# TThuraya/multimodal-PL

Measured on AMD Instinct MI355X. Metric: train voxels/sec at 96^3 patch, 1/2/4/8 MI355X; fwd+bwd step ms, higher is better.
Workload: dtype bf16; 1 GPU; unet3D_baseline([1,2,2,2,2],16,weight_std) fwd+EDiceLoss_partial+bwd+SGD; model=unet3D_baseline-16, global_batch=2, seq_len=884736, parallelism=dp1, world_size_seen=1, force_buckets=False

## Files before the change

multimodal-pl_amd/csrc/conv_brick_gen.hip:

```cpp
#include "common.h"

namespace u3d {

typedef __attribute__((ext_vector_type(8))) __bf16 bf16x8;

constexpr int GB_BD = 4, GB_BH = 8, GB_BW = 16;
constexpr int GB_HD = GB_BD + 2, GB_HH = GB_BH + 2, GB_HW = GB_BW + 2;
constexpr int GB_NH = GB_HD * GB_HH * GB_HW;
constexpr int GB_NT = 512;
constexpr int GB_HLD = (GB_NH + GB_NT / 4 - 1) / (GB_NT / 4);
constexpr int GB_PS = GB_NH * 16 + 64;
constexpr int GB_MAXN = 16;
constexpr int GB_MAXC = 256;

struct GBGeom {
  int n, d, h, w;
  int cin, cout, cin_p, cout_p;
  int nbd, nbh, nbw;
  int gn_groups;
  int nct;
  float* fstats;
  unsigned* fcnt;
};

__device__ __forceinline__ int gb_seg(int r) {
  return (r < 4 || (r >= 12 && r < 16) || (r >= 20 && r < 28)) ? 0 : 1;
}
__device__ __forceinline__ int gb_pos(int r) {
  if (r < 4) return r;
  if (r < 12) return r - 4;
  if (r < 16) return r - 8;
  if (r < 20) return r - 8;
  if (r < 28) return r - 12;
  return r - 16;
}

template <int CO, bool FLIP>
__global__ __launch_bounds__(GB_NT, 1) void convg_brick_kernel(const bf16* __restrict__ x, const bf16* __restrict__ wpk,
                                                              bf16* __restrict__ y, const bf16* __restrict__ res,
                                                              const float* __restrict__ gstat,
                                                              const float* __restrict__ gamma,
                                                              const float* __restrict__ beta, GBGeom g) {
  constexpr int TN = CO / 32;
  constexpr int WROWS = 9 * CO;
  constexpr int WLD = (WROWS * 4 + GB_NT - 1) / GB_NT;
  __shared__ __attribute__((aligned(16))) char hal[4 * GB_PS];
  __shared__ __attribute__((aligned(16))) char wbuf[2][4 * WROWS * 16];

  const int tid = threadIdx.x, lane = tid & 63, wave = tid >> 6;
  const int r = lane & 31, hh = lane >> 5;
  const int nwg = gridDim.x, nct = g.nct;
  int bid;
  {
    const int q = nwg >> 3, rr = nwg & 7, xcd = blockIdx.x & 7, loc = blockIdx.x >> 3;
    bid = (xcd < rr ? xcd * (q + 1) : rr * (q + 1) + (xcd - rr) * q) + loc;
  }
  int b = bid / nct;
  const int bw_ = b % g.nbw; b /= g.nbw;
  const int bh_ = b % g.nbh; b /= g.nbh;
  const int bd_ = b % g.nbd;
  const int nn = b / g.nbd;
  const int d0 = bd_ * GB_BD, h0 = bh_ * GB_BH, w0 = bw_ * GB_BW;
  const int co0 = (bid - (bid / nct) * nct) * CO;
  const bool has_gn = gstat != nullptr;
  const int nchunk = g.cin_p / 32;
  const int nsteps = nchunk * 3;

  u32x4 hpre[GB_HLD];
  u32x4 wpre[WLD];

  const int sch = tid & 3, srow0 = tid >> 2;
  f32x2 sc[4], sh[4];
  auto halo_load = [&](int c) {
#pragma unroll
    for (int i = 0; i < GB_HLD; ++i) {
      const int row = srow0 + i * (GB_NT / 4);
      u32x4 v = {0u, 0u, 0u, 0u};
      if (row < GB_NH) {
        const int hw = row % GB_HW, hr = (row / GB_HW) % GB_HH, hd = row / (GB_HW * GB_HH);
        const int zd = d0 - 1 + hd, zh = h0 - 1 + hr, zw = w0 - 1 + hw;
        const int cc = c * 32 + sch * 8;
        if ((unsigned)zd < (unsigned)g.d && (unsigned)zh < (unsigned)g.h && (unsigned)zw < (unsigned)g.w && cc < g.cin)
          v = *reinterpret_cast<const u32x4*>(x + ((((long long)nn * g.d + zd) * g.h + zh) * g.w + zw) * g.cin + cc);
      }
      hpre[i] = v;
    }
  };
  auto gn_table = [&](int c) {
    if (has_gn) gn_coef8(gstat, gamma, beta, g.gn_groups, g.cin, nn, c * 32 + sch * 8, sc, sh);
  };
  auto halo_commit = [&]() {
#pragma unroll
    for (int i = 0; i < GB_HLD; ++i) {
      const int row = srow0 + i * (GB_NT / 4);
      if (row < GB_NH) {
        u32x4 v = hpre[i];
        if (has_gn) {
          const int hw = row % GB_HW, hr = (row / GB_HW) % GB_HH, hd = row / (GB_HW * GB_HH);
          const int zd = d0 - 1 + hd, zh = h0 - 1 + hr, zw = w0 - 1 + hw;
          if ((unsigned)zd < (unsigned)g.d && (unsigned)zh < (unsigned)g.h && (unsigned)zw < (unsigned)g.w)
            v = gn_relu8(v, sc, sh);
        }
        *reinterpret_cast<u32x4*>(hal + sch * GB_PS + row * 16) = v;
      }
    }
  };
  auto w_load = [&](int s) {
    const int c = s / 3, td = s % 3;
#pragma unroll
    for (int i = 0; i < WLD; ++i) {
      const int ci = tid + i * GB_NT;
      u32x4 v = {0u, 0u, 0u, 0u};
      if (ci < WROWS * 4) {
        const int ch = ci / WROWS, row = ci % WROWS;
        const int j = row / CO, co = co0 + row % CO;
        const int t = td * 9 + j;
        if (co < g.cout_p)
          v = *reinterpret_cast<const u32x4*>(wpk + ((long long)t * g.cout_p + co) * g.cin_p + c * 32 + ch * 8);
      }
      wpre[i] = v;
    }
  };
  auto w_commit = [&](int buf) {
#pragma unroll
    for (int i = 0; i < WLD; ++i) {
      const int ci = tid + i * GB_NT;
      if (ci < WROWS * 4) {
        const int ch = ci / WROWS, row = ci % WROWS;
        *reinterpret_cast<u32x4*>(wbuf[buf] + (ch * WROWS + row) * 16) = wpre[i];
      }
    }
  };

  gn_table(0);
  halo_load(0);
  w_load(0);
  __syncthreads();
  halo_commit();
  w_commit(0);
  __syncthreads();

  f32x16 acc[2][TN];
#pragma unroll
  for (int tm = 0; tm < 2; ++tm)
#pragma unroll
    for (int tn = 0; tn < TN; ++tn)
#pragma unroll
      for (int e = 0; e < 16; ++e) acc[tm][tn][e] = 0.f;

  int arow[2];
#pragma unroll
  for (int tm = 0; tm < 2; ++tm) {
    const int rt = 2 * wave + tm, vd = rt >> 2, vh = 2 * (rt & 3) + gb_seg(r);
    arow[tm] = (vd * GB_HH + vh) * GB_HW + gb_pos(r);
  }

  for (int s = 0; s < nsteps; ++s) {
    const int td = s % 3;
    const bool last_plane = td == 2;
    if (s + 1 < nsteps) w_load(s + 1);
    if (last_plane && s + 1 < nsteps) halo_load(s / 3 + 1);
    const char* wb = wbuf[s & 1];
    const int od = FLIP ? 2 - td : td;
#pragma unroll 3
    for (int j = 0; j < 9; ++j) {
      const int th = j / 3, tw = j % 3;
      const int oh = FLIP ? 2 - th : th, ow = FLIP ? 2 - tw : tw;
      const int toff = (od * GB_HH + oh) * GB_HW + ow;
#pragma unroll
      for (int k = 0; k < 2; ++k) {
        const int plane = 2 * k + hh;
        bf16x8 a[2], bb[TN];
#pragma unroll
        for (int tm = 0; tm < 2; ++tm)
          a[tm] = *reinterpret_cast<const bf16x8*>(hal + plane * GB_PS + (arow[tm] + toff) * 16);
#pragma unroll
        for (int tn = 0; tn < TN; ++tn)
          bb[tn] = *reinterpret_cast<const bf16x8*>(wb + (plane * WROWS + j * CO + tn * 32 + r) * 16);
#pragma unroll
        for (int tm = 0; tm < 2; ++tm)
#pragma unroll
          for (int tn = 0; tn < TN; ++tn)
            acc[tm][tn] = __builtin_amdgcn_mfma_f32_32x32x16_bf16(a[tm], bb[tn], acc[tm][tn], 0, 0, 0);
      }
    }
    if (s + 1 < nsteps) {
      w_commit((s + 1) & 1);
      if (last_plane) {
        gn_table(s / 3 + 1);
        __syncthreads();
        halo_commit();
      }
    }
    __syncthreads();
  }

  constexpr int VB = CO * 2;
  char* const ept = hal + wave * (2 * 32 * VB);
  u32x4 rv[2][VB / 32];
  long long obase[2];
  bool dok[2];
#pragma unroll
  for (int tm = 0; tm < 2; ++tm) {
    const int rt = 2 * wave + tm, zd = d0 + (rt >> 2);
    dok[tm] = zd < g.d;
    obase[tm] = (((long long)nn * g.d + zd) * g.h + h0 + 2 * (rt & 3)) * g.w + w0;
  }
  auto chunk_ok = [&](int tm, int q, long long& off) {
    const int v = q / (VB / 16), c = q % (VB / 16);
    const int seg = v >> 4, pos = v & 15;
    const int rt = 2 * wave + tm, zh = h0 + 2 * (rt & 3) + seg, zw = w0 + pos, co = co0 + c * 8;
    off = (obase[tm] + (long long)seg * g.w + pos) * g.cout + co;
    return dok[tm] && zh < g.h && zw < g.w && co < g.cout;
  };
  if (res) {
#pragma unroll
    for (int tm = 0; tm < 2; ++tm)
#pragma unroll
      for (int u = 0; u < VB / 32; ++u) {
        long long off;
        rv[tm][u] = chunk_ok(tm, lane + 64 * u, off) ? *reinterpret_cast<const u32x4*>(res + off)
                                                      : u32x4{0u, 0u, 0u, 0u};
      }
  }
#pragma unroll
  for (int tm = 0; tm < 2; ++tm)
#pragma unroll
    for (int tn = 0; tn < TN; ++tn)
#pragma unroll
      for (int i = 0; i < 16; ++i) {
        const int ri = (i & 3) + 8 * (i >> 2) + 4 * hh;
        const int v = gb_seg(ri) * 16 + gb_pos(ri);
        *reinterpret_cast<bf16*>(ept + (tm * 32 + v) * VB + (tn * 32 + r) * 2) = from_f<bf16>(acc[tm][tn][i]);
      }
  __builtin_amdgcn_wave_barrier();
  asm volatile("" ::: "memory");
#pragma unroll
  for (int tm = 0; tm < 2; ++tm)
#pragma unroll
    for (int u = 0; u < VB / 32; ++u) {
      const int q = lane + 64 * u;
      long long off;
      if (!chunk_ok(tm, q, off)) continue;
      u32x4 v = *reinterpret_cast<const u32x4*>(ept + tm * 32 * VB + q * 16);
      if (res) {
        float a[8], c[8];
        load16<bf16>(reinterpret_cast<const bf16*>(&v), a);
        load16<bf16>(reinterpret_cast<const bf16*>(&rv[tm][u]), c);
#pragma unroll
        for (int e = 0; e < 8; ++e) a[e] += c[e];
        store16<bf16>(reinterpret_cast<bf16*>(&v), a);
      }
      *reinterpret_cast<u32x4*>(y + off) = v;
    }
}

template <int CO, bool FLIP, int BWX = 16, bool GB = false>
__global__ __launch_bounds__(GB_NT, 1) void convg_pbrick_kernel(const bf16* __restrict__ x, const bf16* __restrict__ wpk,
                                                               bf16* __restrict__ y, const bf16* __restrict__ res,
                                                               const float* __restrict__ gstat,
                                                               const float* __restrict__ gamma,
                                                               const float* __restrict__ beta, GBGeom g, int per,
                                                               int nunits, float* __restrict__ spart = nullptr) {
  constexpr int TN = CO / 32;
  constexpr int WROWS = 9 * CO;
  constexpr int WLD = (WROWS * 4 + GB_NT - 1) / GB_NT;
  constexpr int BW = BWX, HH = GB_BH + 2, HW = BW + 2, NH = (GB_BD + 2) * HH * HW;
  constexpr int HLD = (NH + GB_NT / 4 - 1) / (GB_NT / 4), PS = NH * 16 + 64, TM = BW / 8;
  static_assert(BW == 16 || BW == 8, "brick width");
  auto tile_vox = [](int rt, int r, int& vd, int& vh, int& vw) {
    if constexpr (BW == 16) {
      vd = rt >> 2; vh = 2 * (rt & 3) + gb_seg(r); vw = gb_pos(r);
    } else {
      vd = rt >> 1; vh = 4 * (rt & 1) + (r >> 3); vw = r & 7;
    }
  };
  __shared__ __attribute__((aligned(16))) char hal[4 * PS];
  constexpr int WPS = WROWS * 16 + 64;
  __shared__ __attribute__((aligned(16))) char wbuf[2][4 * WPS];
  __shared__ __attribute__((aligned(16))) f32x2 gtab[2][GB_MAXC];
  __shared__ __attribute__((aligned(16))) f32x4 gbt[GB ? 2 : 1][GB ? GB_MAXC : 1];
  __shared__ double sst[8][2][TN * 2 * 4][2];

  static_assert(!GB || FLIP, "GB: data gradient only");
  constexpr int GB_EARLY = TM == 1 ? TN : 1;
  if constexpr (FLIP && !GB) {
    res = nullptr;
    spart = nullptr;
  }
  float* const gbpart = GB ? spart : nullptr;
  if constexpr (GB) spart = nullptr;
  const int tid = threadIdx.x, lane = tid & 63, wave = tid >> 6;
  const int r = lane & 31, hh = lane >> 5;
  int bid;
  {
    const int nwg = gridDim.x, q = nwg >> 3, rr = nwg & 7, xcd = blockIdx.x & 7, loc = blockIdx.x >> 3;
    bid = (xcd < rr ? xcd * (q + 1) : rr * (q + 1) + (xcd - rr) * q) + loc;
  }
  const int u_begin = bid * per, u_end = min(nunits, u_begin + per);
  const int nct = g.nct;
  const bool has_gn = gstat != nullptr;
  const bool pro_gn = !FLIP && has_gn;
  const int gtc = FLIP ? g.cout : g.cin, gtc_p = FLIP ? g.cout_p : g.cin_p;
  const int nchunk = g.cin_p / 32;
  const int nsteps = nchunk * 3;

  struct Unit {
    int nn, d0, h0, w0, co0;
  };
  auto unit_geo = [&](int u) {
    Unit q;
    int b = u / nct;
    q.co0 = (u - b * nct) * CO;
    const int bw_ = b % g.nbw; b /= g.nbw;
    const int bh_ = b % g.nbh; b /= g.nbh;
    const int bd_ = b % g.nbd;
    q.nn = b / g.nbd;
    q.d0 = bd_ * GB_BD; q.h0 = bh_ * GB_BH; q.w0 = bw_ * BW;
    return q;
  };

  u32x4 hpre[HLD];
  unsigned hmask = 0;
  u32x4 wpre[WLD];
  const int sch = tid & 3, srow0 = tid >> 2;
  int stg_nn = 0, stg_c = 0;
  const auto srs = __builtin_amdgcn_make_buffer_rsrc((void*)gstat, 0, has_gn ? 0x7FFFFFFF : 0, 0x00020000);
  const auto grs = __builtin_amdgcn_make_buffer_rsrc((void*)gamma, 0, has_gn ? 0x7FFFFFFF : 0, 0x00020000);
  const auto brs = __builtin_amdgcn_make_buffer_rsrc((void*)beta, 0, has_gn ? 0x7FFFFFFF : 0, 0x00020000);
  auto gtab_fill = [&](int nn) {
    if (has_gn && tid < gtc_p) {
      int t = tid;
      asm volatile("" : "+v"(t));
      const int c = min(t, gtc - 1), gg = c / (gtc / g.gn_groups);
      const int so = (nn * g.gn_groups + gg) * 8;
      const float mean = __builtin_bit_cast(float, __builtin_amdgcn_raw_buffer_load_b32(srs, so, 0, 0));
      const float rstd = __builtin_bit_cast(float, __builtin_amdgcn_raw_buffer_load_b32(srs, so + 4, 0, 0));
      const float sc_ = rstd * __builtin_bit_cast(float, __builtin_amdgcn_raw_buffer_load_b32(grs, c * 4, 0, 0));
      const float sh_ = __builtin_bit_cast(float, __builtin_amdgcn_raw_buffer_load_b32(brs, c * 4, 0, 0)) - mean * sc_;
      if constexpr (GB)
        gbt[nn & 1][tid] = f32x4{sc_, sh_, rstd, mean};
      else
        gtab[nn & 1][tid] = f32x2{sc_, sh_};
    }
  };
  const int xbytes = g.n * g.d * g.h * g.w * g.cin * 2, ybytes = g.n * g.d * g.h * g.w * g.cout * 2;
  const auto xrs = __builtin_amdgcn_make_buffer_rsrc((void*)x, 0, xbytes, 0x00020000);
  const auto wrs = __builtin_amdgcn_make_buffer_rsrc((void*)wpk, 0, 27 * g.cout_p * g.cin_p * 2, 0x00020000);
  const auto rrs = __builtin_amdgcn_make_buffer_rsrc((void*)res, 0, res ? ybytes : 0, 0x00020000);
  const auto yrs = __builtin_amdgcn_make_buffer_rsrc((void*)y, 0, ybytes, 0x00020000);
  const auto prs = __builtin_amdgcn_make_buffer_rsrc((void*)spart, 0, spart ? 0x7FFFFFFF : 0, 0x00020000);
  auto halo_load = [&](const Unit& q, int c) {
    hmask = 0;
    stg_nn = q.nn;
    stg_c = c;
    const int cc = c * 32 + sch * 8;
#pragma unroll
    for (int i = 0; i < HLD; ++i) {
      const int row = srow0 + i * (GB_NT / 4);
      const int hw = row % HW, hr = (row / HW) % HH, hd = row / (HW * HH);
      const int zd = q.d0 - 1 + hd, zh = q.h0 - 1 + hr, zw = q.w0 - 1 + hw;
      const bool in = row < NH && (unsigned)zd < (unsigned)g.d && (unsigned)zh < (unsigned)g.h &&
                      (unsigned)zw < (unsigned)g.w;
      hmask |= (in ? 1u : 0u) << i;
      const unsigned off =
          in && cc < g.cin ? (unsigned)(((((q.nn * g.d + zd) * g.h + zh) * g.w + zw) * g.cin + cc) * 2) : 0xFFFFFFF0u;
      hpre[i] = __builtin_bit_cast(u32x4, __builtin_amdgcn_raw_buffer_load_b128(xrs, off, 0, 0));
    }
  };
  auto halo_commit = [&]() {
    f32x2 sc[4], sh[4];
    if (pro_gn) {
      const f32x2* t = &gtab[stg_nn & 1][stg_c * 32 + sch * 8];
#pragma unroll
      for (int e = 0; e < 4; ++e) {
        const f32x2 a0 = t[2 * e], a1 = t[2 * e + 1];
        sc[e] = f32x2{a0[0], a1[0]};
        sh[e] = f32x2{a0[1], a1[1]};
      }
    }
#pragma unroll
    for (int i = 0; i < HLD; ++i) {
      const int row = srow0 + i * (GB_NT / 4);
      if (row < NH) {
        u32x4 v = hpre[i];
        if (pro_gn && ((hmask >> i) & 1u)) v = gn_relu8(v, sc, sh);
        *reinterpret_cast<u32x4*>(hal + sch * PS + row * 16) = v;
      }
    }
  };
  auto w_load = [&](int co0, int s) {
    const int c = s / 3, td = s % 3;
#pragma unroll
    for (int i = 0; i < WLD; ++i) {
      const int ci = tid + i * GB_NT;
      const int ch = ci & 3, row = ci >> 2;
      const int j = row / CO, co = co0 + row % CO;
      const int t = td * 9 + j;
      const unsigned off = ci < WROWS * 4 && co < g.cout_p
                               ? (unsigned)(((t * g.cout_p + co) * g.cin_p + c * 32 + ch * 8) * 2) : 0xFFFFFFF0u;
      wpre[i] = __builtin_bit_cast(u32x4, __builtin_amdgcn_raw_buffer_load_b128(wrs, off, 0, 0));
    }
  };
// ... 397 lines not shown

static bool pbrick_bw8(int w) {
  const int e8 = opt(OPT_CONVG_BW8);
  return e8 >= 0 ? e8 != 0 : (w % 16 != 0 && w % 8 == 0);
}

static bool gb_co64(long long units, int cout, int cout_p) {
  const int env_co32 = opt(OPT_CONVG_CO32);
  if (cout_p < 64 || env_co32 == 1) return false;
  return !(env_co32 < 0 && units * cdiv(cout, 64) < 128 && units * cdiv(cout, 32) >= 128);
}

struct GBPlan {
  bool pers, bw8, co64;
  int nunits, per, nwg;
};

static GBPlan gb_plan(bool flip, int n, int cin, int d, int h, int w, int cout, bool gn, bool residual, bool gbparts,
                      GBGeom& g) {
  g = GBGeom{};
  g.n = n; g.d = d; g.h = h; g.w = w;
  g.cin = cin; g.cout = cout; g.cin_p = round_up(cin, 32); g.cout_p = round_up(cout, 32);
  GBPlan p{};
  p.pers = opt(OPT_CONVG_PERSIST) != 0 && n >= 1 && n <= GB_MAXN &&
           fits_buffer_offsets((long long)n * d * h * w * std::max(cin, cout) * 2) &&
           fits_buffer_offsets(27LL * g.cout_p * g.cin_p * 2) &&
           (!gn || (gbparts ? g.cout_p : g.cin_p) <= GB_MAXC) && !(flip && residual);
  p.bw8 = p.pers && pbrick_bw8(w);
  g.nbd = cdiv(d, GB_BD); g.nbh = cdiv(h, GB_BH); g.nbw = cdiv(w, p.bw8 ? 8 : GB_BW);
  const long long bricks = (long long)n * g.nbd * g.nbh * g.nbw;
  p.co64 = gb_co64(bricks, cout, g.cout_p);
  g.nct = cdiv(cout, p.co64 ? 64 : 32);
  p.nunits = (int)(bricks * g.nct);
  p.per = p.pers ? cdiv(p.nunits, convg_num_cus()) : 1;
  p.nwg = cdiv(p.nunits, p.per);
  return p;
}

extern "C" long long u3d_convg_brick_stats_ws_floats(int n, int d, int h, int w, int cout) {
  return (long long)n * cdiv(d, GB_BD) * cdiv(h, GB_BH) * cdiv(w, 8) * cdiv(cout, 32) * 128;
}

struct GBArgs {
  const void *x, *wpk;
  void* y;
  const void* res;
  const float *gstat, *gamma, *beta;
  float* spart;
  hipStream_t s;
};

template <int CO, bool FLIP, int BWX, bool GB>
static void gb_launch(const GBPlan& p, const GBGeom& g, const GBArgs& a) {
  if (p.pers)
    hipLaunchKernelGGL((convg_pbrick_kernel<CO, FLIP, BWX, GB>), dim3(p.nwg), dim3(GB_NT), 0, a.s, (const bf16*)a.x,
                       (const bf16*)a.wpk, (bf16*)a.y, (const bf16*)a.res, a.gstat, a.gamma, a.beta, g, p.per, p.nunits,
                       a.spart);
  else
    hipLaunchKernelGGL((convg_brick_kernel<CO, FLIP>), dim3(p.nwg), dim3(GB_NT), 0, a.s, (const bf16*)a.x,
                       (const bf16*)a.wpk, (bf16*)a.y, (const bf16*)a.res, a.gstat, a.gamma, a.beta, g);
}

template <int CO>
static void gb_dispatch(bool flip, bool gb, const GBPlan& p, const GBGeom& g, const GBArgs& a) {
  if (!flip) p.bw8 ? gb_launch<CO, false, 8, false>(p, g, a) : gb_launch<CO, false, 16, false>(p, g, a);
  else if (gb) p.bw8 ? gb_launch<CO, true, 8, true>(p, g, a) : gb_launch<CO, true, 16, true>(p, g, a);
  else p.bw8 ? gb_launch<CO, true, 8, false>(p, g, a) : gb_launch<CO, true, 16, false>(p, g, a);
}

static int convg_impl(int flip, const void* x, int n, int cin, int d, int h, int w, const void* wpk, int cout,
                      const float* gn_stats, const float* gn_gamma, const float* gn_beta, int gn_groups,
                      const void* residual, void* y, float* spart, float* stats_out, u3d_stream_t stream,
                      const void* gbx = nullptr, float* gbparts = nullptr, unsigned* fcnt = nullptr) {
  U3D_REQUIRE(x && wpk && y && n >= 1 && n <= GB_MAXN, "convg_brick: bad args");
  U3D_REQUIRE(!gbparts || (flip && gbx && gn_stats && !residual && !spart && cout % gn_groups == 0),
              "convg_brick_dgrad_gn: bad args");
  U3D_REQUIRE(cin % 8 == 0 && cout % 8 == 0, "convg_brick: channels must be multiples of 8");
  U3D_REQUIRE(!gn_stats || (gn_gamma && gn_beta && gn_groups > 0 && (gbparts ? cout : cin) % gn_groups == 0),
              "convg_brick: bad GN");
  GBGeom g;
  const GBPlan p = gb_plan(flip, n, cin, d, h, w, cout, gn_stats, residual, gbparts, g);
  g.gn_groups = gn_groups;
  U3D_REQUIRE(!spart || (p.pers && !flip && cout % 32 == 0), "convg_brick_stats: needs the persistent forward, cout %% 32 == 0");
  U3D_REQUIRE(!gbparts || p.pers, "convg_brick_dgrad_gn: needs the persistent data gradient (u3d_convg_brick_gn_nparts)");
  if (spart && fcnt) {
    g.fstats = stats_out;
    g.fcnt = fcnt;
  }
  hipStream_t s = (hipStream_t)stream;
  const GBArgs a{x, wpk, y, gbparts ? gbx : residual, gn_stats, gn_gamma, gn_beta, gbparts ? gbparts : spart, s};
  if (p.co64) gb_dispatch<64>(flip, gbparts, p, g, a);
  else gb_dispatch<32>(flip, gbparts, p, g, a);
  int rc = check_launch(p.pers ? "convg_pbrick_kernel" : "convg_brick_kernel");
  if (rc || !spart || fcnt) return rc;
  hipLaunchKernelGGL(pbrick_gn_finalize_kernel, dim3(n * 16), dim3(256), 0, s, (const double*)spart, p.co64 ? 64 : 32, g.nct,
                     g.nbd * g.nbh * g.nbw, cout, (double)(cout / 16) * d * h * w, stats_out);
  return check_launch("pbrick_gn_finalize_kernel");
}

extern "C" int u3d_convg_brick(int flip, const void* x, int n, int cin, int d, int h, int w, const void* wpk, int cout,
                               const float* gn_stats, const float* gn_gamma, const float* gn_beta, int gn_groups,
                               const void* residual, void* y, u3d_stream_t stream) {
  return convg_impl(flip, x, n, cin, d, h, w, wpk, cout, gn_stats, gn_gamma, gn_beta, gn_groups, residual, y, nullptr,
                    nullptr, stream);
}

extern "C" int u3d_convg_brick_gn_nparts(int n, int cin, int d, int h, int w, int cout) {
  GBGeom g;
// ... 33 lines not shown
```

Before: 336.6 million voxels/s.

## Switch brick conv kernels to 16x16x32 MFMA with swizzled LDS layout

Reworks the brick convolution kernels to use 16x16x32 bf16 MFMA tiles instead of 32x32x16. Each wave now covers four rows of 16 voxels, and the halo and weight LDS buffers get padded or XOR-swizzled strides to cut bank conflicts. The epilogue and the GroupNorm stats reduction are rewritten around the new fragment layout, using permlane swaps and bpermute trees. The old 32x32 path is kept as a separate kernel for the 8-wide bricks. This is a large change that risks register pressure and correctness problems in the new reduction paths.

Result: no change. 338.4 million voxels/s, median of 6 (+0.5%).

```diff
diff --git a/multimodal-pl_amd/csrc/conv_brick_gen.hip b/multimodal-pl_amd/csrc/conv_brick_gen.hip
--- a/multimodal-pl_amd/csrc/conv_brick_gen.hip
+++ b/multimodal-pl_amd/csrc/conv_brick_gen.hip
@@ -9,7 +9,8 @@
 constexpr int GB_NH = GB_HD * GB_HH * GB_HW;
 constexpr int GB_NT = 512;
 constexpr int GB_HLD = (GB_NH + GB_NT / 4 - 1) / (GB_NT / 4);
-constexpr int GB_PS = GB_NH * 16 + 64;
+constexpr int gb_plane_stride(int nh) { return (nh * 16 + 255) / 256 * 256 + 32; }
+constexpr int GB_PS = gb_plane_stride(GB_NH);
 constexpr int GB_MAXN = 16;
 constexpr int GB_MAXC = 256;
 
@@ -23,16 +24,48 @@
   unsigned* fcnt;
 };
 
-__device__ __forceinline__ int gb_seg(int r) {
-  return (r < 4 || (r >= 12 && r < 16) || (r >= 20 && r < 28)) ? 0 : 1;
-}
-__device__ __forceinline__ int gb_pos(int r) {
-  if (r < 4) return r;
-  if (r < 12) return r - 4;
-  if (r < 16) return r - 8;
-  if (r < 20) return r - 8;
-  if (r < 28) return r - 12;
-  return r - 16;
+__device__ __forceinline__ int gb_m16(int l16) { return (l16 >= 4 && l16 < 12) ? 2 * (l16 - 4) : 2 * (l16 & 7) + 1; }
+
+__device__ __forceinline__ int gb_wswz(int plane) { return 2 * (plane & 1) + 12 * (plane >> 1); }
+
+template <int NV, int NC, int LD>
+__device__ __forceinline__ void gb_mfma_tap(f32x4 (*acc)[LD], int c0, const bf16x8 (&fw)[NC], const bf16x8 (&fx)[NV]) {
+#pragma unroll
+  for (int v = 0; v < NV; ++v)
+#pragma unroll
+    for (int cb = 0; cb < NC; ++cb)
+      acc[v][c0 + cb] = __builtin_amdgcn_mfma_f32_16x16x32_bf16(fw[cb], fx[v], acc[v][c0 + cb], 0, 0, 0);
+}
+
+__device__ __forceinline__ int gb_cbase(int q4) { return 16 * (q4 & 1) + 8 * (q4 >> 1); }
+__device__ __forceinline__ u32x4 gb_pack_pair(const f32x4& a0, const f32x4& a1) {
+  uint32_t pk[2][2] = {{pack_bf16x2(a0[0], a0[1]), pack_bf16x2(a0[2], a0[3])},
+                       {pack_bf16x2(a1[0], a1[1]), pack_bf16x2(a1[2], a1[3])}};
+#pragma unroll
+  for (int e = 0; e < 2; ++e) {
+    const auto sw = __builtin_amdgcn_permlane16_swap(pk[0][e], pk[1][e], false, false);
+    pk[0][e] = sw[0];
+    pk[1][e] = sw[1];
+  }
+  return u32x4{pk[0][0], pk[0][1], pk[1][0], pk[1][1]};
+}
+
+__device__ __forceinline__ void gb_tree_lanes(int lane, int m, int (&px)[5]) {
+  constexpr int C[5] = {8, 12, 4, 2, 1};
+#pragma unroll
+  for (int k = 0; k < 5; ++k) {
+    const int t = m ^ C[k], h = t >> 1;
+    px[k] = ((lane & 48) + ((t & 1) ? (h < 4 ? h : h + 8) : h + 4)) * 4;
+  }
+}
+__device__ __forceinline__ float gb_bperm(int addr, float v) {
+  return __builtin_bit_cast(float, __builtin_amdgcn_ds_bpermute(addr, __builtin_bit_cast(int, v)));
+}
+__device__ __forceinline__ float gb_wave_tree(float y0, float y1, const int (&px)[5]) {
+  float t = y0 + gb_bperm(px[0], y1);
+#pragma unroll
+  for (int k = 1; k < 5; ++k) t += gb_bperm(px[k], t);
+  return t;
 }
 
 template <int CO, bool FLIP>
@@ -41,14 +74,14 @@
                                                               const float* __restrict__ gstat,
                                                               const float* __restrict__ gamma,
                                                               const float* __restrict__ beta, GBGeom g) {
-  constexpr int TN = CO / 32;
+  constexpr int NVB = 4, NCB = CO / 16;
   constexpr int WROWS = 9 * CO;
   constexpr int WLD = (WROWS * 4 + GB_NT - 1) / GB_NT;
   __shared__ __attribute__((aligned(16))) char hal[4 * GB_PS];
   __shared__ __attribute__((aligned(16))) char wbuf[2][4 * WROWS * 16];
 
   const int tid = threadIdx.x, lane = tid & 63, wave = tid >> 6;
-  const int r = lane & 31, hh = lane >> 5;
+  const int l16 = lane & 15, q4 = lane >> 4;
   const int nwg = gridDim.x, nct = g.nct;
   int bid;
   {
@@ -140,20 +173,13 @@
   w_commit(0);
   __syncthreads();
 
-  f32x16 acc[2][TN];
-#pragma unroll
-  for (int tm = 0; tm < 2; ++tm)
-#pragma unroll
-    for (int tn = 0; tn < TN; ++tn)
-#pragma unroll
-      for (int e = 0; e < 16; ++e) acc[tm][tn][e] = 0.f;
-
-  int arow[2];
-#pragma unroll
-  for (int tm = 0; tm < 2; ++tm) {
-    const int rt = 2 * wave + tm, vd = rt >> 2, vh = 2 * (rt & 3) + gb_seg(r);
-    arow[tm] = (vd * GB_HH + vh) * GB_HW + gb_pos(r);
-  }
+  f32x4 acc[NVB][NCB];
+#pragma unroll
+  for (int vb = 0; vb < NVB; ++vb)
+#pragma unroll
+    for (int cb = 0; cb < NCB; ++cb) acc[vb][cb] = f32x4{0.f, 0.f, 0.f, 0.f};
+
+  const int xrow = ((wave >> 1) * GB_HH + 4 * (wave & 1)) * GB_HW + gb_m16(l16);
 
   for (int s = 0; s < nsteps; ++s) {
     const int td = s % 3;
@@ -167,22 +193,14 @@
       const int th = j / 3, tw = j % 3;
       const int oh = FLIP ? 2 - th : th, ow = FLIP ? 2 - tw : tw;
       const int toff = (od * GB_HH + oh) * GB_HW + ow;
-#pragma unroll
-      for (int k = 0; k < 2; ++k) {
-        const int plane = 2 * k + hh;
-        bf16x8 a[2], bb[TN];
-#pragma unroll
-        for (int tm = 0; tm < 2; ++tm)
-          a[tm] = *reinterpret_cast<const bf16x8*>(hal + plane * GB_PS + (arow[tm] + toff) * 16);
-#pragma unroll
-        for (int tn = 0; tn < TN; ++tn)
-          bb[tn] = *reinterpret_cast<const bf16x8*>(wb + (plane * WROWS + j * CO + tn * 32 + r) * 16);
-#pragma unroll
-        for (int tm = 0; tm < 2; ++tm)
-#pragma unroll
-          for (int tn = 0; tn < TN; ++tn)
-            acc[tm][tn] = __builtin_amdgcn_mfma_f32_32x32x16_bf16(a[tm], bb[tn], acc[tm][tn], 0, 0, 0);
-      }
+      bf16x8 fx[NVB], fw[NCB];
+#pragma unroll
+      for (int vb = 0; vb < NVB; ++vb)
+        fx[vb] = *reinterpret_cast<const bf16x8*>(hal + q4 * GB_PS + (xrow + toff + vb * GB_HW) * 16);
+#pragma unroll
+      for (int cb = 0; cb < NCB; ++cb)
+        fw[cb] = *reinterpret_cast<const bf16x8*>(wb + (q4 * WROWS + j * CO + cb * 16 + l16) * 16);
+      gb_mfma_tap<NVB, NCB>(acc, 0, fw, fx);
     }
     if (s + 1 < nsteps) {
       w_commit((s + 1) & 1);
@@ -196,63 +214,51 @@
   }
 
   constexpr int VB = CO * 2;
-  char* const ept = hal + wave * (2 * 32 * VB);
-  u32x4 rv[2][VB / 32];
-  long long obase[2];
-  bool dok[2];
-#pragma unroll
-  for (int tm = 0; tm < 2; ++tm) {
-    const int rt = 2 * wave + tm, zd = d0 + (rt >> 2);
-    dok[tm] = zd < g.d;
-    obase[tm] = (((long long)nn * g.d + zd) * g.h + h0 + 2 * (rt & 3)) * g.w + w0;
-  }
-  auto chunk_ok = [&](int tm, int q, long long& off) {
-    const int v = q / (VB / 16), c = q % (VB / 16);
-    const int seg = v >> 4, pos = v & 15;
-    const int rt = 2 * wave + tm, zh = h0 + 2 * (rt & 3) + seg, zw = w0 + pos, co = co0 + c * 8;
-    off = (obase[tm] + (long long)seg * g.w + pos) * g.cout + co;
-    return dok[tm] && zh < g.h && zw < g.w && co < g.cout;
+  constexpr int NCH = VB / 16;
+  char* const ept = hal + wave * (64 * VB);
+  u32x4 rv[NCH];
+  const int zd = d0 + (wave >> 1), zh0 = h0 + 4 * (wave & 1);
+  const long long obase = (((long long)nn * g.d + zd) * g.h + zh0) * g.w + w0;
+  auto chunk_ok = [&](int q, long long& off) {
+    const int v = q / NCH, c = q % NCH;
+    const int vb = v >> 4, pos = v & 15, co = co0 + c * 8;
+    off = (obase + (long long)vb * g.w + pos) * g.cout + co;
+    return zd < g.d && zh0 + vb < g.h && w0 + pos < g.w && co < g.cout;
   };
   if (res) {
 #pragma unroll
-    for (int tm = 0; tm < 2; ++tm)
-#pragma unroll
-      for (int u = 0; u < VB / 32; ++u) {
-        long long off;
-        rv[tm][u] = chunk_ok(tm, lane + 64 * u, off) ? *reinterpret_cast<const u32x4*>(res + off)
-                                                      : u32x4{0u, 0u, 0u, 0u};
-      }
-  }
-#pragma unroll
-  for (int tm = 0; tm < 2; ++tm)
-#pragma unroll
-    for (int tn = 0; tn < TN; ++tn)
-#pragma unroll
-      for (int i = 0; i < 16; ++i) {
-        const int ri = (i & 3) + 8 * (i >> 2) + 4 * hh;
-        const int v = gb_seg(ri) * 16 + gb_pos(ri);
-        *reinterpret_cast<bf16*>(ept + (tm * 32 + v) * VB + (tn * 32 + r) * 2) = from_f<bf16>(acc[tm][tn][i]);
-      }
+    for (int u = 0; u < NCH; ++u) {
+      long long off;
+      rv[u] = chunk_ok(lane + 64 * u, off) ? *reinterpret_cast<const u32x4*>(res + off) : u32x4{0u, 0u, 0u, 0u};
+    }
+  }
+  const int m16 = gb_m16(l16);
+#pragma unroll
+  for (int vb = 0; vb < NVB; ++vb)
+#pragma unroll
+    for (int cb = 0; cb < NCB; ++cb) {
+      const f32x4 a = acc[vb][cb];
+      *reinterpret_cast<uint2*>(ept + (vb * 16 + m16) * VB + (cb * 16 + 4 * q4) * 2) =
+          uint2{pack_bf16x2(a[0], a[1]), pack_bf16x2(a[2], a[3])};
+    }
   __builtin_amdgcn_wave_barrier();
   asm volatile("" ::: "memory");
 #pragma unroll
-  for (int tm = 0; tm < 2; ++tm)
-#pragma unroll
-    for (int u = 0; u < VB / 32; ++u) {
-      const int q = lane + 64 * u;
-      long long off;
-      if (!chunk_ok(tm, q, off)) continue;
-      u32x4 v = *reinterpret_cast<const u32x4*>(ept + tm * 32 * VB + q * 16);
-      if (res) {
-        float a[8], c[8];
-        load16<bf16>(reinterpret_cast<const bf16*>(&v), a);
-        load16<bf16>(reinterpret_cast<const bf16*>(&rv[tm][u]), c);
-#pragma unroll
-        for (int e = 0; e < 8; ++e) a[e] += c[e];
-        store16<bf16>(reinterpret_cast<bf16*>(&v), a);
-      }
-      *reinterpret_cast<u32x4*>(y + off) = v;
-    }
+  for (int u = 0; u < NCH; ++u) {
+    const int q = lane + 64 * u;
+    long long off;
+    if (!chunk_ok(q, off)) continue;
+    u32x4 v = *reinterpret_cast<const u32x4*>(ept + q * 16);
+    if (res) {
+      float a[8], c[8];
+      load16<bf16>(reinterpret_cast<const bf16*>(&v), a);
+      load16<bf16>(reinterpret_cast<const bf16*>(&rv[u]), c);
+#pragma unroll
+      for (int e = 0; e < 8; ++e) a[e] += c[e];
+      store16<bf16>(reinterpret_cast<bf16*>(&v), a);
+    }
+    *reinterpret_cast<u32x4*>(y + off) = v;
+  }
 }
 
 template <int CO, bool FLIP, int BWX = 16, bool GB = false>
@@ -262,28 +268,25 @@
                                                                const float* __restrict__ gamma,
                                                                const float* __restrict__ beta, GBGeom g, int per,
                                                                int nunits, float* __restrict__ spart = nullptr) {
-  constexpr int TN = CO / 32;
+  constexpr int TN = CO / 32, NCB = CO / 16;
   constexpr int WROWS = 9 * CO;
   constexpr int WLD = (WROWS * 4 + GB_NT - 1) / GB_NT;
   constexpr int BW = BWX, HH = GB_BH + 2, HW = BW + 2, NH = (GB_BD + 2) * HH * HW;
-  constexpr int HLD = (NH + GB_NT / 4 - 1) / (GB_NT / 4), PS = NH * 16 + 64, TM = BW / 8;
-  static_assert(BW == 16 || BW == 8, "brick width");
-  auto tile_vox = [](int rt, int r, int& vd, int& vh, int& vw) {
-    if constexpr (BW == 16) {
-      vd = rt >> 2; vh = 2 * (rt & 3) + gb_seg(r); vw = gb_pos(r);
-    } else {
-      vd = rt >> 1; vh = 4 * (rt & 1) + (r >> 3); vw = r & 7;
-    }
+  constexpr int HLD = (NH + GB_NT / 4 - 1) / (GB_NT / 4), PS = gb_plane_stride(NH), NVB = BW / 4, NVH = NVB / 2;
+  static_assert(BW == 16, "brick width");
+  auto tile_vox = [](int wave, int vb, int m, int& vd, int& vh, int& vw) {
+    vd = wave >> 1; vh = 4 * (wave & 1) + vb; vw = m;
   };
   __shared__ __attribute__((aligned(16))) char hal[4 * PS];
-  constexpr int WPS = WROWS * 16 + 64;
+  constexpr int WPS = WROWS * 16;
+  static_assert(WPS % 256 == 0 && WROWS % 16 == 0, "weight plane stride / swizzle blocks");
   __shared__ __attribute__((aligned(16))) char wbuf[2][4 * WPS];
   __shared__ __attribute__((aligned(16))) f32x2 gtab[2][GB_MAXC];
   __shared__ __attribute__((aligned(16))) f32x4 gbt[GB ? 2 : 1][GB ? GB_MAXC : 1];
-  __shared__ double sst[8][2][TN * 2 * 4][2];
+  __shared__ double sst[8][4][TN * 4][2];
 
   static_assert(!GB || FLIP, "GB: data gradient only");
-  constexpr int GB_EARLY = TM == 1 ? TN : 1;
+  constexpr int GB_EARLY = 1;
   if constexpr (FLIP && !GB) {
     res = nullptr;
     spart = nullptr;
@@ -291,7 +294,7 @@
   float* const gbpart = GB ? spart : nullptr;
   if constexpr (GB) spart = nullptr;
   const int tid = threadIdx.x, lane = tid & 63, wave = tid >> 6;
-  const int r = lane & 31, hh = lane >> 5;
+  const int l16 = lane & 15, q4 = lane >> 4, m16 = gb_m16(l16), cbase = gb_cbase(q4);
   int bid;
   {
     const int nwg = gridDim.x, q = nwg >> 3, rr = nwg & 7, xcd = blockIdx.x & 7, loc = blockIdx.x >> 3;
@@ -349,6 +352,472 @@
   const auto wrs = __builtin_amdgcn_make_buffer_rsrc((void*)wpk, 0, 27 * g.cout_p * g.cin_p * 2, 0x00020000);
   const auto rrs = __builtin_amdgcn_make_buffer_rsrc((void*)res, 0, res ? ybytes : 0, 0x00020000);
   const auto yrs = __builtin_amdgcn_make_buffer_rsrc((void*)y, 0, ybytes, 0x00020000);
+  float* const pbase = GB ? gbpart : spart;
+  const auto prs = __builtin_amdgcn_make_buffer_rsrc((void*)pbase, 0, pbase ? 0x7FFFFFFF : 0, 0x00020000);
+  auto halo_load = [&](const Unit& q, int c) {
+    hmask = 0;
+    stg_nn = q.nn;
+    stg_c = c;
+    const int cc = c * 32 + sch * 8;
+#pragma unroll
+    for (int i = 0; i < HLD; ++i) {
+      const int row = srow0 + i * (GB_NT / 4);
+      const int hw = row % HW, hr = (row / HW) % HH, hd = row / (HW * HH);
+      const int zd = q.d0 - 1 + hd, zh = q.h0 - 1 + hr, zw = q.w0 - 1 + hw;
+      const bool in = row < NH && (unsigned)zd < (unsigned)g.d && (unsigned)zh < (unsigned)g.h &&
+                      (unsigned)zw < (unsigned)g.w;
+      hmask |= (in ? 1u : 0u) << i;
+      const unsigned off =
+          in && cc < g.cin ? (unsigned)(((((q.nn * g.d + zd) * g.h + zh) * g.w + zw) * g.cin + cc) * 2) : 0xFFFFFFF0u;
+      hpre[i] = __builtin_bit_cast(u32x4, __builtin_amdgcn_raw_buffer_load_b128(xrs, off, 0, 0));
+    }
+  };
+  auto halo_commit = [&]() {
+    f32x2 sc[4], sh[4];
+    if (pro_gn) {
+      const f32x2* t = &gtab[stg_nn & 1][stg_c * 32 + sch * 8];
+#pragma unroll
+      for (int e = 0; e < 4; ++e) {
+        const f32x2 a0 = t[2 * e], a1 = t[2 * e + 1];
+        sc[e] = f32x2{a0[0], a1[0]};
+        sh[e] = f32x2{a0[1], a1[1]};
+      }
+    }
+#pragma unroll
+    for (int i = 0; i < HLD; ++i) {
+      const int row = srow0 + i * (GB_NT / 4);
+      if (row < NH) {
+        u32x4 v = hpre[i];
+        if (pro_gn && ((hmask >> i) & 1u)) v = gn_relu8(v, sc, sh);
+        *reinterpret_cast<u32x4*>(hal + sch * PS + row * 16) = v;
+      }
+    }
+  };
+  auto w_load = [&](int co0, int s) {
+    const int c = s / 3, td = s % 3;
+#pragma unroll
+    for (int i = 0; i < WLD; ++i) {
+      const int ci = tid + i * GB_NT;
+      const int ch = ci & 3, row = ci >> 2;
+      const int j = row / CO, co = co0 + row % CO;
+      const int t = td * 9 + j;
+      const unsigned off = ci < WROWS * 4 && co < g.cout_p
+                               ? (unsigned)(((t * g.cout_p + co) * g.cin_p + c * 32 + ch * 8) * 2) : 0xFFFFFFF0u;
+      wpre[i] = __builtin_bit_cast(u32x4, __builtin_amdgcn_raw_buffer_load_b128(wrs, off, 0, 0));
+    }
+  };
+  auto w_commit = [&](int buf) {
+#pragma unroll
+    for (int i = 0; i < WLD; ++i) {
+      const int ci = tid + i * GB_NT;
+      if (ci < WROWS * 4) {
+        const int ch = ci & 3, row = ci >> 2;
+        *reinterpret_cast<u32x4*>(wbuf[buf] + ch * WPS + (row ^ gb_wswz(ch)) * 16) = wpre[i];
+      }
+    }
+  };
+
+  int xoff, woff;
+  {
+    int vd, vh, vw;
+    tile_vox(wave, 0, m16, vd, vh, vw);
+    xoff = q4 * PS + ((vd * HH + vh) * HW + vw) * 16;
+    woff = q4 * WPS + (l16 ^ gb_wswz(q4)) * 16;
+  }
+
+  Unit cu = unit_geo(u_begin);
+  gtab_fill(cu.nn);
+  __syncthreads();
+  halo_load(cu, 0);
+  w_load(cu.co0, 0);
+  halo_commit();
+  w_commit(0);
+  __syncthreads();
+  int par = 0;
+
+  for (int u = u_begin; u < u_end; ++u) {
+    const bool more = u + 1 < u_end;
+    const Unit nu = more ? unit_geo(u + 1) : cu;
+    if (more && nu.nn != cu.nn) gtab_fill(nu.nn);
+    f32x4 acc[NVB][NCB];
+#pragma unroll
+    for (int vb = 0; vb < NVB; ++vb)
+#pragma unroll
+      for (int cb = 0; cb < NCB; ++cb) acc[vb][cb] = f32x4{0.f, 0.f, 0.f, 0.f};
+    int ovox[NVB];
+    bool ook[NVB];
+    auto out_vox = [&]() {
+#pragma unroll
+      for (int vb = 0; vb < NVB; ++vb) {
+        int vd, vh, vw;
+        tile_vox(wave, vb, m16, vd, vh, vw);
+        const int zd = cu.d0 + vd, zh = cu.h0 + vh, zw = cu.w0 + vw;
+        ook[vb] = zd < g.d && zh < g.h && zw < g.w;
+        ovox[vb] = ((cu.nn * g.d + zd) * g.h + zh) * g.w + zw;
+      }
+    };
+    if constexpr (GB) out_vox();
+    u32x4 rv[NVB][TN];
+    auto res_load = [&](int tn) {
+      const int co = cu.co0 + tn * 32 + cbase;
+#pragma unroll
+      for (int vb = 0; vb < NVB; ++vb) {
+        const unsigned ro = (ook[vb] && co < g.cout) ? (unsigned)((ovox[vb] * g.cout + co) * 2) : 0xFFFFFFF0u;
+        rv[vb][tn] = __builtin_bit_cast(u32x4, __builtin_amdgcn_raw_buffer_load_b128(rrs, ro, 0, 0));
+      }
+    };
+    for (int s = 0; s < nsteps; ++s) {
+      const int td = s % 3;
+      const bool last = s + 1 == nsteps;
+      const bool next = !last || more;
+      if (next) {
+        const Unit& lq = last ? nu : cu;
+        w_load(lq.co0, last ? 0 : s + 1);
+        if (td == 2) halo_load(lq, last ? 0 : s / 3 + 1);
+      }
+      if constexpr (GB) {
+        if (last)
+#pragma unroll
+          for (int tn = 0; tn < GB_EARLY; ++tn) res_load(tn);
+      }
+      const char* wb = wbuf[par] + woff;
+      const int od = FLIP ? 2 - td : td;
+      const char* xb = hal + xoff + od * (HH * HW * 16);
+      auto rd_w = [&](bf16x8* dst, int j, int cb0, int nc) {
+#pragma unroll
+        for (int c = 0; c < nc; ++c)
+          dst[c] = *reinterpret_cast<const bf16x8*>(wb + (j * CO + (cb0 + c) * 16) * 16);
+      };
+      auto rd_x = [&](bf16x8* dst, int j, int vb0, int nv) {
+        const int th = j / 3, tw = j % 3;
+        const int oh = FLIP ? 2 - th : th, ow = FLIP ? 2 - tw : tw;
+#pragma unroll
+        for (int v = 0; v < nv; ++v)
+          dst[v] = *reinterpret_cast<const bf16x8*>(xb + (oh * HW + ow + (vb0 + v) * HW) * 16);
+      };
+      if constexpr (NVB * NCB == 16) {
+        constexpr int NCH = NCB / 2;
+        bf16x8 fw[2][NCH], fx[2][NVH];
+        rd_x(fx[0], 0, 0, NVH);
+        rd_w(fw[0], 0, 0, NCH);
+        static_for<0, 36>([&](auto ic) {
+          constexpr int t = decltype(ic)::value, j = t >> 2, qi = t & 3, qs = (j & 1) ? 3 - qi : qi;
+          constexpr int vh = qs >> 1, ch = (qs & 1) ^ vh;
+          if constexpr (qi == 0) rd_w(fw[(j & 1) ^ 1], j, NCH, NCH);
+          if constexpr (qi == 1) rd_x(fx[1], j, ((j & 1) ? 0 : 1) * NVH, NVH);
+          if constexpr (qi == 2 && j < 8) rd_x(fx[0], j + 1, ((j & 1) ? 0 : 1) * NVH, NVH);
+          if constexpr (qi == 3 && j < 8) rd_w(fw[(j + 1) & 1], j + 1, 0, NCH);
+          __builtin_amdgcn_sched_barrier(0);
+          gb_mfma_tap<NVH, NCH>(acc + vh * NVH, ch * NCH, fw[(j & 1) ^ ch], fx[qi >> 1]);
+          __builtin_amdgcn_sched_barrier(0);
+        });
+      } else {
+        bf16x8 fw[2][NCB], fx[2][NVB];
+        rd_x(fx[0], 0, 0, NVB);
+        rd_w(fw[0], 0, 0, NCB);
+        static_for<0, 9>([&](auto ic) {
+          constexpr int j = decltype(ic)::value;
+          if constexpr (j < 8) {
+            rd_x(fx[(j + 1) & 1], j + 1, 0, NVB);
+            rd_w(fw[(j + 1) & 1], j + 1, 0, NCB);
+          }
+          __builtin_amdgcn_sched_barrier(0);
+          gb_mfma_tap<NVB, NCB>(acc, 0, fw[j & 1], fx[j & 1]);
+          __builtin_amdgcn_sched_barrier(0);
+        });
+      }
+      if (last) break;
+      w_commit(par ^ 1);
+      if (td == 2) {
+        __syncthreads();
+        halo_commit();
+      }
+      __syncthreads();
+      par ^= 1;
+    }
+
+    if constexpr (!GB) out_vox();
+    if (!GB && res) res_load(0);
+    if (more) {
+      w_commit(par ^ 1);
+      __syncthreads();
+      halo_commit();
+    }
+    if (res) {
+#pragma unroll
+      for (int tn = GB ? GB_EARLY : 1; tn < TN; ++tn) res_load(tn);
+    }
+    __syncthreads();
+    par ^= 1;
+    f32x2 ps[2 * 4];
+    float shv[4];
+    float* const gred = reinterpret_cast<float*>(&sst[0][0][0][0]);
+    static_assert(!GB || sizeof(sst) >= 8 * TN * 4 * 16 * sizeof(float), "GB reduction buffer");
+#pragma unroll
+    for (int tn = 0; tn < TN; ++tn) {
+      const int co = cu.co0 + tn * 32 + cbase;
+      if constexpr (GB) {
+        u32x4 o[NVB];
+#pragma unroll
+        for (int vb = 0; vb < NVB; ++vb) {
+          o[vb] = gb_pack_pair(acc[vb][2 * tn], acc[vb][2 * tn + 1]);
+          if (ook[vb] && co < g.cout)
+            __builtin_amdgcn_raw_buffer_store_b128(o[vb], yrs, (unsigned)((ovox[vb] * g.cout + co) * 2), 0, 0);
+        }
+        const f32x4* tb = &gbt[cu.nn & 1][co];
+#pragma unroll
+        for (int vb = 0; vb < NVB; ++vb)
+#pragma unroll
+          for (int k = 0; k < 4; ++k) o[vb][k] = (ook[vb] && co < g.cout) ? o[vb][k] : 0u;
+#pragma unroll
+        for (int e = 0; e < 8; ++e) {
+          int px[5], pm = m16;
+          asm volatile("" : "+v"(pm));
+          gb_tree_lanes(lane, pm, px);
+          const f32x4 t = tb[e];
+          float gbs[2][2] = {{0.f, 0.f}, {0.f, 0.f}};
+#pragma unroll
+          for (int vb = 0; vb < NVB; ++vb) {
+            const uint32_t ow = o[vb][e >> 1], xw = rv[vb][tn][e >> 1];
+            const float a = __builtin_bit_cast(float, (e & 1) ? (ow & 0xFFFF0000u) : (ow << 16));
+            const float xv = __builtin_bit_cast(float, (e & 1) ? (xw & 0xFFFF0000u) : (xw << 16));
+            const float gd = fmaf(xv, t[0], t[1]) > 0.f ? a : 0.f;
+            gbs[vb & 1][0] += gd;
+            gbs[vb & 1][1] = fmaf(gd, xv - t[3], gbs[vb & 1][1]);
+          }
+          const float s0 = gb_wave_tree(gbs[0][0], gbs[1][0], px), s1 = gb_wave_tree(gbs[0][1], gbs[1][1], px);
+          if (l16 < 2) gred[((wave * TN + tn) * 4 + q4) * 16 + e * 2 + l16] = l16 ? s1 : s0;
+        }
+        continue;
+      }
+#pragma unroll
+      for (int i = 0; i < 2 * 4; ++i) ps[i] = f32x2{0.f, 0.f};
+#pragma unroll
+      for (int vb = 0; vb < NVB; ++vb) {
+        u32x4 o = gb_pack_pair(acc[vb][2 * tn], acc[vb][2 * tn + 1]);
+        if (res) {
+          float a8[8], c8[8];
+          load16<bf16>(reinterpret_cast<const bf16*>(&o), a8);
+          load16<bf16>(reinterpret_cast<const bf16*>(&rv[vb][tn]), c8);
+#pragma unroll
+          for (int e = 0; e < 8; ++e) a8[e] += c8[e];
+          store16<bf16>(reinterpret_cast<bf16*>(&o), a8);
+        }
+        if (ook[vb] && co < g.cout)
+          __builtin_amdgcn_raw_buffer_store_b128(o, yrs, (unsigned)((ovox[vb] * g.cout + co) * 2), 0, 0);
+        if (spart != nullptr) {
+          float f8[8];
+          load16<bf16>(reinterpret_cast<const bf16*>(&o), f8);
+          const bool on = ook[vb] && co < g.cout;
+          if (vb == 0)
+#pragma unroll
+            for (int q = 0; q < 4; ++q)
+              shv[q] = __builtin_bit_cast(float, __builtin_amdgcn_ds_bpermute((16 * q4 + 4) * 4,
+                                                                              __builtin_bit_cast(int, f8[2 * q])));
+#pragma unroll
+          for (int q = 0; q < 4; ++q) {
+            const float a0 = f8[2 * q] - shv[q], a1 = f8[2 * q + 1] - shv[q];
+            f32x2& t = ps[(vb & 1) * 4 + q];
+            t[0] += on ? a0 + a1 : 0.f;
+            t[1] = on ? fmaf(a0, a0, fmaf(a1, a1, t[1])) : t[1];
+          }
+        }
+      }
+      if (spart != nullptr) {
+        int px[5], pm = m16;
+        asm volatile("" : "+v"(pm));
+        gb_tree_lanes(lane, pm, px);
+        float t1 = 0.f, t2 = 0.f;
+#pragma unroll
+        for (int q = 0; q < 4; ++q) {
+          const float u1 = gb_wave_tree(ps[q][0], ps[4 + q][0], px), u2 = gb_wave_tree(ps[q][1], ps[4 + q][1], px);
+          t1 = l16 == q ? u1 : t1;
+          t2 = l16 == q ? u2 : t2;
+        }
+        unsigned nvox = 0;
+#pragma unroll
+        for (int vb = 0; vb < NVB; ++vb) {
+          const unsigned long long b = __ballot(ook[vb]);
+          nvox += __builtin_popcount((unsigned)(b >> (16 * q4)) & 0xFFFFu);
+        }
+        if (l16 < 4) {
+          const int i = l16;
+          float shi = shv[0];
+#pragma unroll
+          for (int j = 1; j < 4; ++j) shi = i == j ? shv[j] : shi;
+          const double sh = (double)shi;
+          const double nn = co < g.cout ? 2.0 * nvox : 0.0;
+          sst[wave][q4][tn * 4 + i][0] = (double)t1 + nn * sh;
+          sst[wave][q4][tn * 4 + i][1] = (double)t2 + 2.0 * sh * (double)t1 + nn * sh * sh;
+        }
+      }
+    }
+    if constexpr (GB) {
+      __syncthreads();
+      if (tid < CO * 2) {
+        int ti = tid;
+        asm volatile("" : "+v"(ti));
+        const int cl = ti >> 1, k = ti & 1, tn = cl >> 5, row = ((cl >> 4) & 1) | ((cl >> 2) & 2), e = cl & 7;
+        float t = 0.f;
+#pragma unroll
+        for (int w = 0; w < 8; ++w) t += gred[((w * TN + tn) * 4 + row) * 16 + e * 2 + k];
+        const int co = cu.co0 + cl;
+        if (co < g.cout)
+          __builtin_amdgcn_raw_buffer_store_b32(__builtin_bit_cast(unsigned, k ? t * gbt[cu.nn & 1][co][2] : t), prs,
+                                                (((u / nct) * g.cout + co) * 2 + k) * 4, 0, 0);
+      }
+    }
+    if (spart != nullptr) {
+      __syncthreads();
+      if (tid < CO / 2) {
+        const int c = 2 * tid, tn = c >> 5, row = ((c >> 4) & 1) | ((c >> 2) & 2), q = (c & 7) >> 1;
+        double t0 = 0.0, t1 = 0.0;
+        for (int w = 0; w < 8; ++w) {
+          t0 += sst[w][row][tn * 4 + q][0];
+          t1 += sst[w][row][tn * 4 + q][1];
+        }
+        typedef __attribute__((ext_vector_type(2))) double f64x2;
+        if (g.fcnt)
+          __builtin_amdgcn_raw_buffer_store_b128(__builtin_bit_cast(u32x4, (f64x2){t0, t1}), prs, (u * CO + c) * 8, 0,
+                                                 16);
+        else
+          __builtin_amdgcn_raw_buffer_store_b128(__builtin_bit_cast(u32x4, (f64x2){t0, t1}), prs, (u * CO + c) * 8, 0,
+                                                 0);
+      }
+    }
+    cu = nu;
+  }
+  if constexpr (!GB) {
+    if (spart != nullptr && g.fcnt != nullptr) {
+      if (last_arriver(g.fcnt, gridDim.x)) {
+        const int bps = g.nbd * g.nbh * g.nbw, cpg = g.cout / 16, l16 = tid & 15;
+        const double m = (double)cpg * g.d * g.h * g.w;
+        for (int p0 = 0; p0 < g.n * 16; p0 += GB_NT / 16) {
+          const int p = p0 + (tid >> 4);
+          double s1 = 0, s2 = 0;
+          if (p < g.n * 16) {
+            typedef __attribute__((ext_vector_type(2))) double f64x2;
+            const int nn = p >> 4, gr = p & 15, ncp = cpg >> 1, nk = (bps - l16 + 15) / 16 * ncp;
+            for (int k0 = 0; k0 < nk; k0 += 8) {
+              f64x2 q[8];
+#pragma unroll
+              for (int u = 0; u < 8; ++u) {
+                const int k = k0 + u, bi = k / ncp, c = gr * cpg + 2 * (k - bi * ncp), ct = c / CO, cl = c - ct * CO;
+                const long long brick = (long long)nn * bps + l16 + 16 * bi;
+                q[u] = __builtin_bit_cast(f64x2, __builtin_amdgcn_raw_buffer_load_b128(
+                                                     prs, k < nk ? (int)(((brick * g.nct + ct) * CO + cl) * 8)
+                                                                 : (int)0xFFFFFFF0u, 0, 16));
+              }
+#pragma unroll
+              for (int u = 0; u < 8; ++u)
+                if (k0 + u < nk) {
+                  s1 += q[u][0];
+                  s2 += q[u][1];
+                }
+            }
+          }
+#pragma unroll
+          for (int o = 8; o > 0; o >>= 1) {
+            s1 += __shfl_xor(s1, o);
+            s2 += __shfl_xor(s2, o);
+          }
+          if (p < g.n * 16 && l16 == 0) gn_store_stats(g.fstats + p * 2, s1, s2, m);
+        }
+      }
+    }
+  }
+}
+
+template <int CO, bool FLIP, int BWX = 8, bool GB = false>
+__global__ __launch_bounds__(GB_NT, 1) void convg_pbrick32_kernel(const bf16* __restrict__ x, const bf16* __restrict__ wpk,
+                                                               bf16* __restrict__ y, const bf16* __restrict__ res,
+                                                               const float* __restrict__ gstat,
+                                                               const float* __restrict__ gamma,
+                                                               const float* __restrict__ beta, GBGeom g, int per,
+                                                               int nunits, float* __restrict__ spart = nullptr) {
+  constexpr int TN = CO / 32;
+  constexpr int WROWS = 9 * CO;
+  constexpr int WLD = (WROWS * 4 + GB_NT - 1) / GB_NT;
+  constexpr int BW = BWX, HH = GB_BH + 2, HW = BW + 2, NH = (GB_BD + 2) * HH * HW;
+  constexpr int HLD = (NH + GB_NT / 4 - 1) / (GB_NT / 4), PS = NH * 16 + 64, TM = BW / 8;
+  static_assert(BW == 8, "the 32x32x16 form runs the 8-wide bricks only");
+  auto tile_vox = [](int rt, int r, int& vd, int& vh, int& vw) {
+    vd = rt >> 1; vh = 4 * (rt & 1) + (r >> 3); vw = r & 7;
+  };
+  __shared__ __attribute__((aligned(16))) char hal[4 * PS];
+  constexpr int WPS = WROWS * 16 + 64;
+  __shared__ __attribute__((aligned(16))) char wbuf[2][4 * WPS];
+  __shared__ __attribute__((aligned(16))) f32x2 gtab[2][GB_MAXC];
+  __shared__ __attribute__((aligned(16))) f32x4 gbt[GB ? 2 : 1][GB ? GB_MAXC : 1];
+  __shared__ double sst[8][2][TN * 2 * 4][2];
+
+  static_assert(!GB || FLIP, "GB: data gradient only");
+  constexpr int GB_EARLY = TM == 1 ? TN : 1;
+  if constexpr (FLIP && !GB) {
+    res = nullptr;
+    spart = nullptr;
+  }
+  float* const gbpart = GB ? spart : nullptr;
+  if constexpr (GB) spart = nullptr;
+  const int tid = threadIdx.x, lane = tid & 63, wave = tid >> 6;
+  const int r = lane & 31, hh = lane >> 5;
+  int bid;
+  {
+    const int nwg = gridDim.x, q = nwg >> 3, rr = nwg & 7, xcd = blockIdx.x & 7, loc = blockIdx.x >> 3;
+    bid = (xcd < rr ? xcd * (q + 1) : rr * (q + 1) + (xcd - rr) * q) + loc;
+  }
+  const int u_begin = bid * per, u_end = min(nunits, u_begin + per);
+  const int nct = g.nct;
+  const bool has_gn = gstat != nullptr;
+  const bool pro_gn = !FLIP && has_gn;
+  const int gtc = FLIP ? g.cout : g.cin, gtc_p = FLIP ? g.cout_p : g.cin_p;
+  const int nchunk = g.cin_p / 32;
+  const int nsteps = nchunk * 3;
+
+  struct Unit {
+    int nn, d0, h0, w0, co0;
+  };
+  auto unit_geo = [&](int u) {
+    Unit q;
+    int b = u / nct;
+    q.co0 = (u - b * nct) * CO;
+    const int bw_ = b % g.nbw; b /= g.nbw;
+    const int bh_ = b % g.nbh; b /= g.nbh;
+    const int bd_ = b % g.nbd;
+    q.nn = b / g.nbd;
+    q.d0 = bd_ * GB_BD; q.h0 = bh_ * GB_BH; q.w0 = bw_ * BW;
+    return q;
+  };
+
+  u32x4 hpre[HLD];
+  unsigned hmask = 0;
+  u32x4 wpre[WLD];
+  const int sch = tid & 3, srow0 = tid >> 2;
+  int stg_nn = 0, stg_c = 0;
+  const auto srs = __builtin_amdgcn_make_buffer_rsrc((void*)gstat, 0, has_gn ? 0x7FFFFFFF : 0, 0x00020000);
+  const auto grs = __builtin_amdgcn_make_buffer_rsrc((void*)gamma, 0, has_gn ? 0x7FFFFFFF : 0, 0x00020000);
+  const auto brs = __builtin_amdgcn_make_buffer_rsrc((void*)beta, 0, has_gn ? 0x7FFFFFFF : 0, 0x00020000);
+  auto gtab_fill = [&](int nn) {
+    if (has_gn && tid < gtc_p) {
+      int t = tid;
+      asm volatile("" : "+v"(t));
+      const int c = min(t, gtc - 1), gg = c / (gtc / g.gn_groups);
+      const int so = (nn * g.gn_groups + gg) * 8;
+      const float mean = __builtin_bit_cast(float, __builtin_amdgcn_raw_buffer_load_b32(srs, so, 0, 0));
+      const float rstd = __builtin_bit_cast(float, __builtin_amdgcn_raw_buffer_load_b32(srs, so + 4, 0, 0));
+      const float sc_ = rstd * __builtin_bit_cast(float, __builtin_amdgcn_raw_buffer_load_b32(grs, c * 4, 0, 0));
+      const float sh_ = __builtin_bit_cast(float, __builtin_amdgcn_raw_buffer_load_b32(brs, c * 4, 0, 0)) - mean * sc_;
+      if constexpr (GB)
+        gbt[nn & 1][tid] = f32x4{sc_, sh_, rstd, mean};
+      else
+        gtab[nn & 1][tid] = f32x2{sc_, sh_};
+    }
+  };
+  const int xbytes = g.n * g.d * g.h * g.w * g.cin * 2, ybytes = g.n * g.d * g.h * g.w * g.cout * 2;
+  const auto xrs = __builtin_amdgcn_make_buffer_rsrc((void*)x, 0, xbytes, 0x00020000);
+  const auto wrs = __builtin_amdgcn_make_buffer_rsrc((void*)wpk, 0, 27 * g.cout_p * g.cin_p * 2, 0x00020000);
+  const auto rrs = __builtin_amdgcn_make_buffer_rsrc((void*)res, 0, res ? ybytes : 0, 0x00020000);
+  const auto yrs = __builtin_amdgcn_make_buffer_rsrc((void*)y, 0, ybytes, 0x00020000);
   const auto prs = __builtin_amdgcn_make_buffer_rsrc((void*)spart, 0, spart ? 0x7FFFFFFF : 0, 0x00020000);
   auto halo_load = [&](const Unit& q, int c) {
     hmask = 0;
@@ -852,8 +1321,12 @@
 
 template <int CO, bool FLIP, int BWX, bool GB>
 static void gb_launch(const GBPlan& p, const GBGeom& g, const GBArgs& a) {
-  if (p.pers)
-    hipLaunchKernelGGL((convg_pbrick_kernel<CO, FLIP, BWX, GB>), dim3(p.nwg), dim3(GB_NT), 0, a.s, (const bf16*)a.x,
+  if (p.pers && BWX == 16)
+    hipLaunchKernelGGL((convg_pbrick_kernel<CO, FLIP, 16, GB>), dim3(p.nwg), dim3(GB_NT), 0, a.s, (const bf16*)a.x,
+                       (const bf16*)a.wpk, (bf16*)a.y, (const bf16*)a.res, a.gstat, a.gamma, a.beta, g, p.per, p.nunits,
+                       a.spart);
+  else if (p.pers)
+    hipLaunchKernelGGL((convg_pbrick32_kernel<CO, FLIP, 8, GB>), dim3(p.nwg), dim3(GB_NT), 0, a.s, (const bf16*)a.x,
                        (const bf16*)a.wpk, (bf16*)a.y, (const bf16*)a.res, a.gstat, a.gamma, a.beta, g, p.per, p.nunits,
                        a.spart);
   else
```
